# JuliaMolSim/DFTK.jl

Hardware: AMD Instinct MI355X
Metric: SCF iterations/sec (Hψ applies/sec) at fixed Ecut·atoms (higher is better)
Workload: dtype f64

## Files before the change

### dftk.jl_amd/_lib.py

```python
from __future__ import annotations

import ctypes as C
import os

from . import _build

c_cplx_p = C.c_void_p
_i64 = C.c_int64


class dftk_mi_cplx(C.Structure):
    _fields_ = [("re", C.c_double), ("im", C.c_double)]


class dftk_mi_batch_op(C.Structure):
    _fields_ = ([(name, C.c_int32) for name in ("type", "fiber", "trans", "m", "k", "i0", "mode", "flags", "join_next",
                                                 "sync_after", "status", "reserved")] +
                [(name, _i64) for name in ("n", "gm", "gn", "gk", "lda", "ldb", "ldc")] +
                [("alpha", dftk_mi_cplx), ("beta", dftk_mi_cplx), ("s0", C.c_double)] +
                [(name, C.c_void_p) for name in ("A", "B", "W", "W2", "W3", "C", "D", "E", "F", "kb", "host")] +
                [("bytes", C.c_uint64)])


class DftkMiError(RuntimeError):
# ... 87 lines not shown
    "dftk_mi_cube_gradient": (C.c_int, [C.c_void_p, C.c_void_p, C.c_void_p, C.c_void_p]),
    "dftk_mi_xc_gga_spin": (C.c_int, [C.c_void_p, _i64, C.c_void_p, C.c_void_p, C.c_int, C.c_double, C.c_void_p, C.c_void_p,
                                      C.c_void_p]),
    "dftk_mi_symmetrize_rho": (C.c_int, [C.c_void_p, C.c_int, C.c_void_p, C.c_void_p, C.c_int, C.c_void_p, C.c_void_p]),
    "dftk_mi_mix_kerker": (C.c_int, [C.c_void_p, C.c_void_p, C.c_double, C.c_void_p, C.c_void_p]),
    "dftk_mi_mix_dielectric": (C.c_int, [C.c_void_p, C.c_void_p, C.c_double, C.c_double, C.c_void_p, C.c_void_p]),
    "dftk_mi_chi0_dielectric_apply": (C.c_int, [C.c_void_p, C.c_void_p, C.c_double, C.c_double, C.c_void_p, C.c_void_p]),
    "dftk_mi_cube_fourier_filter": (C.c_int, [C.c_void_p, C.c_void_p, C.c_void_p, C.c_void_p]),
    "dftk_mi_kblocks_set_potential": (C.c_int, [C.c_int, C.c_void_p, C.c_void_p]),
    "dftk_mi_lobpcg_multi": (C.c_int, [C.c_int, C.c_void_p, C.c_int, C.c_void_p, C.c_void_p, C.c_double, C.c_int, C.c_int,
                                       C.c_int, C.c_int, C.c_void_p, C.c_void_p, C.c_void_p, C.c_void_p, C.c_void_p,
                                       C.c_void_p, C.c_void_p]),
    "dftk_mi_density_accumulate_multi": (C.c_int, [C.c_int, C.c_void_p, C.c_void_p, C.c_void_p, C.c_void_p, C.c_void_p,
                                                   C.c_void_p]),
    "dftk_mi_density_accumulate_multi2": (C.c_int, [C.c_int, C.c_void_p, C.c_void_p, C.c_void_p, C.c_void_p, C.c_void_p,
                                                    C.c_void_p, C.c_void_p, C.c_void_p]),
    "dftk_mi_band_kinetic_multi": (C.c_int, [C.c_int, C.c_void_p, C.c_void_p, C.c_void_p, C.c_void_p, C.c_void_p]),
    "dftk_mi_batch_stats": (C.c_int, [C.POINTER(_i64), C.POINTER(_i64), C.POINTER(_i64), C.POINTER(_i64)]),
    "dftk_mi_lobpcg_small_stats": (C.c_int, [C.POINTER(_i64), C.POINTER(_i64)]),
    "dftk_mi_ortho_small": (C.c_int, [C.c_void_p, _i64, C.c_int, C.c_void_p, _i64, C.c_int, C.c_void_p, _i64, C.c_void_p,
                                      C.c_double, C.c_void_p]),
    "dftk_mi_batch_replay": (C.c_int, [C.c_void_p, C.c_int, C.c_int, C.c_void_p]),
    "dftk_mi_lobpcg_last_AX": (C.c_void_p, [C.c_void_p]),
    "dftk_mi_lobpcg_history": (C.c_int, [C.c_void_p, C.POINTER(C.c_int), C.POINTER(C.c_int), C.c_void_p, C.c_size_t,
                                         C.POINTER(C.c_int)]),
    "dftk_mi_columnwise_norms": (C.c_int, [C.c_void_p, _i64, C.c_int, C.c_void_p, _i64, C.c_void_p]),
    "dftk_mi_columnwise_dots": (C.c_int, [C.c_void_p, _i64, C.c_int, C.c_void_p, _i64, C.c_void_p, _i64, C.c_void_p]),
    "dftk_mi_ortho_qr": (C.c_int, [C.c_void_p, _i64, C.c_int, C.c_void_p, _i64, C.c_int, C.POINTER(C.c_int),
                                   C.POINTER(C.c_int)]),
    "dftk_mi_tpa_precondprep": (C.c_int, [C.c_void_p, C.c_int, C.c_void_p, _i64, C.c_void_p]),
    "dftk_mi_tpa_ldiv": (C.c_int, [C.c_void_p, C.c_int, C.c_void_p, _i64, C.c_void_p, C.c_double, C.c_void_p, _i64]),
    "dftk_mi_block_residual": (C.c_int, [C.c_void_p, C.c_int, C.c_void_p, _i64, C.c_void_p, _i64, C.c_void_p,
                                         C.c_void_p, _i64, C.c_void_p, C.c_void_p, C.c_void_p]),
    "dftk_mi_kblock_set_gamma_real": (C.c_int, [C.c_void_p, C.c_int]),
    "dftk_mi_gamma_half_size": (C.c_int, [C.c_void_p, C.POINTER(_i64)]),
    "dftk_mi_gamma_tables_host": (C.c_int, [C.c_int, C.c_int, C.c_int, _i64, C.c_void_p, C.POINTER(_i64), C.c_void_p,
                                            C.c_void_p]),
    "dftk_mi_gamma_compress": (C.c_int, [C.c_void_p, C.c_int, C.c_void_p, _i64, C.c_void_p, _i64]),
    "dftk_mi_gamma_compress_aligned": (C.c_int, [C.c_void_p, C.c_int, C.c_void_p, _i64, C.c_void_p, _i64]),
    "dftk_mi_gamma_expand": (C.c_int, [C.c_void_p, C.c_int, C.c_void_p, _i64, C.c_void_p, _i64]),
    "dftk_mi_gamma_apply_H": (C.c_int, [C.c_void_p, C.c_int, C.c_int, C.c_void_p, _i64, C.c_void_p, _i64]),
    "dftk_mi_density_accumulate_real": (C.c_int, [C.c_void_p, C.c_int, C.c_void_p, _i64, C.c_void_p, C.c_void_p]),
    "dftk_mi_shard_plan_host": (C.c_int, [C.c_int, C.c_int, C.c_int, C.c_void_p, C.c_void_p, C.c_void_p, C.c_void_p,
                                          C.c_void_p, C.c_void_p]),
    "dftk_mi_kblock_set_shard": (C.c_int, [C.c_void_p, C.c_void_p, C.c_void_p]),
    "dftk_mi_zgemm": (C.c_int, [C.c_void_p, C.c_char, _i64, _i64, _i64, dftk_mi_cplx, C.c_void_p, _i64,
                                C.c_void_p, _i64, dftk_mi_cplx, C.c_void_p, _i64]),
    "dftk_mi_zgemm_ex": (C.c_int, [C.c_void_p, C.c_char, _i64, _i64, _i64, dftk_mi_cplx, C.c_void_p, _i64,
                                   C.c_void_p, _i64, dftk_mi_cplx, C.c_void_p, _i64, C.c_int]),
    "dftk_mi_zgemm_to": (C.c_int, [C.c_void_p, C.c_char, _i64, _i64, _i64, dftk_mi_cplx, C.c_void_p, _i64,
                                   C.c_void_p, _i64, dftk_mi_cplx, C.c_void_p, _i64, C.c_void_p, C.c_int]),
    "dftk_mi_zgemm_plan_host": (C.c_int, [C.c_char, _i64, _i64, _i64, C.c_int, C.POINTER(C.c_int)]),
    "dftk_mi_zgemm_fold_host": (C.c_int, [C.c_char, _i64, _i64, _i64, C.c_int, C.c_int, C.POINTER(C.c_int), C.POINTER(C.c_int)]),
    "dftk_mi_heev": (C.c_int, [C.c_void_p, C.c_int, C.c_void_p, _i64, C.c_void_p, C.c_void_p, _i64]),
    "dftk_mi_prof_zgemm_shapes": (C.c_int, [C.c_void_p, C.c_int, C.c_void_p, C.c_void_p, C.POINTER(C.c_int)]),
    "dftk_mi_eig_mirror_tall": (C.c_int, [C.c_void_p, C.c_int, C.c_int, C.c_void_p, _i64]),
    "dftk_mi_heev_lowest": (C.c_int, [C.c_void_p, C.c_int, C.c_int, C.c_void_p, _i64, C.c_void_p, C.c_void_p, _i64]),
    "dftk_mi_heev_sigma_host": (C.c_int, [C.c_int, C.c_void_p, C.c_int, C.POINTER(C.c_double), C.POINTER(C.c_double),
                                          C.POINTER(C.c_int), C.c_double]),
    "dftk_mi_potrf_trtri": (C.c_int, [C.c_void_p, C.c_int, C.c_void_p, _i64, C.c_void_p, _i64]),
    "dftk_mi_potrf_trtri_real": (C.c_int, [C.c_void_p, C.c_int, C.c_void_p, _i64, C.c_void_p, _i64]),
    "dftk_mi_lowdin_ortho": (C.c_int, [C.c_void_p, _i64, C.c_int, C.c_void_p, _i64, C.c_void_p]),
    "dftk_mi_pdos_accumulate": (C.c_int, [C.c_void_p, _i64, C.c_int, C.c_void_p, _i64, C.c_int, C.c_void_p, _i64, C.c_void_p,
                                          C.c_double, C.c_int, C.c_double, C.c_int, C.c_void_p, C.c_void_p, C.c_void_p]),
    "dftk_mi_hubbard_occupation": (C.c_int, [C.c_void_p, _i64, C.c_int, C.c_void_p, _i64, C.c_int, C.c_void_p, _i64, C.c_void_p,
                                             C.c_int, C.c_void_p, C.c_void_p, C.c_void_p]),
    "dftk_mi_hubbard_rotate": (C.c_int, [C.c_void_p, _i64, C.c_int, C.c_void_p, C.c_void_p, C.c_void_p, _i64, C.c_void_p,
                                         C.c_void_p, _i64]),
    "dftk_mi_comm_get_unique_id": (C.c_int, [C.c_char_p]),
    "dftk_mi_comm_init_rank": (C.c_int, [C.c_char_p, C.c_int, C.c_int, C.c_int, C.POINTER(C.c_void_p)]),
    "dftk_mi_comm_create_host": (C.c_int, [C.c_int, C.c_int, C.c_int, C.c_void_p, C.c_void_p, C.c_void_p,
                                           C.POINTER(C.c_void_p)]),
    "dftk_mi_comm_destroy": (C.c_int, [C.c_void_p]),
    "dftk_mi_comm_describe": (C.c_int, [C.c_void_p, C.POINTER(C.c_int), C.POINTER(C.c_int), C.POINTER(C.c_int)]),
    "dftk_mi_comm_rank": (C.c_int, [C.c_void_p]),
    "dftk_mi_comm_size": (C.c_int, [C.c_void_p]),
    "dftk_mi_allreduce_sum_f64": (C.c_int, [C.c_void_p, C.c_void_p, C.c_size_t, C.c_void_p]),
    "dftk_mi_prof_enable": (C.c_int, [C.c_void_p, C.c_int]),
    "dftk_mi_prof_get": (C.c_int, [C.c_void_p, C.c_int, C.POINTER(C.c_double), C.POINTER(C.c_double),
                                   C.POINTER(_i64)]),
    "dftk_mi_anderson_create": (C.c_int, [C.c_void_p, _i64, C.c_int, C.c_double, C.c_double, C.POINTER(C.c_void_p)]),
    "dftk_mi_anderson_destroy": (C.c_int, [C.c_void_p]),
    "dftk_mi_anderson_reset": (C.c_int, [C.c_void_p]),
    "dftk_mi_anderson_history": (C.c_int, [C.c_void_p]),
    "dftk_mi_anderson_step": (C.c_int, [C.c_void_p, C.c_void_p, C.c_double, C.c_void_p, C.c_void_p, C.POINTER(C.c_int)]),
    "dftk_mi_chi0_mix": (C.c_int, [C.c_void_p, C.c_int, C.c_void_p, C.c_void_p, C.c_void_p, C.c_double, C.c_int, C.c_double,
                                   C.c_double, C.c_void_p, C.c_double, C.c_int, C.c_int, C.c_void_p, C.POINTER(C.c_int),
                                   C.POINTER(C.c_int)]),
    "dftk_mi_launch_count": (C.c_int, [C.POINTER(_i64), C.POINTER(_i64)]),
    "dftk_mi_device_buffers_live": (C.c_int, [C.POINTER(_i64), C.POINTER(_i64)]),
    "dftk_mi_kblock_reuse_AX": (C.c_int, [C.c_void_p, C.c_int]),
    "dftk_mi_ax_reuse_count": (C.c_int, [C.POINTER(_i64)]),
    "dftk_mi_planes_reuse_count": (C.c_int, [C.POINTER(_i64)]),
    "dftk_mi_step_sums": (C.c_int, [C.c_void_p, _i64, C.c_void_p, C.c_void_p, C.c_void_p, C.c_void_p]),
    "dftk_mi_fermi_bisection": (C.c_int, [C.c_int, C.c_void_p, C.c_void_p, C.c_void_p, C.c_int, C.c_double, C.c_double,
                                          C.c_double, C.c_double, C.c_double, C.POINTER(C.c_double)]),
    "dftk_mi_diag_mfma_peak": (C.c_int, [C.c_void_p, C.c_int, C.c_int, C.POINTER(C.c_double)]),
    "dftk_mi_jacobi_schedule_host": (C.c_int, [C.c_int, C.c_int, C.POINTER(C.c_int), C.POINTER(C.c_int),
                                               C.POINTER(C.c_int)]),
    "dftk_mi_fft_plan_host": (C.c_int, [C.c_int, C.POINTER(C.c_int), C.POINTER(C.c_int), C.POINTER(C.c_int)]),
    "dftk_mi_sphere_tables_host": (C.c_int, [C.c_int, C.c_int, C.c_int, _i64, C.c_void_p, C.POINTER(_i64),
                                             C.POINTER(C.c_int), C.c_void_p, C.c_void_p]),
}

ALLREDUCE_FN = C.CFUNCTYPE(C.c_int, C.c_void_p, C.POINTER(C.c_double), C.c_size_t)
ALLTOALLV_FN = C.CFUNCTYPE(C.c_int, C.c_void_p, C.POINTER(C.c_double), C.POINTER(C.c_size_t), C.POINTER(C.c_size_t),
# ... 38 lines not shown
```

### dftk.jl_amd/csrc/api.cpp

```cpp
#include "common.h"
#include <chrono>
#include "batch.h"
#include <algorithm>
#include <cmath>
#include <cstdarg>
#include <cstdio>
#include <cstdlib>
#include <cstring>
#include <vector>

static thread_local char g_err[1024] = "";

void dftk_set_error(const char* fmt, ...) {
    va_list ap;
    va_start(ap, fmt);
    vsnprintf(g_err, sizeof(g_err), fmt, ap);
    va_end(ap);
}

extern "C" const char* dftk_mi_last_error(void) { return g_err; }

hipError_t dftk_scratch_malloc(void** p, size_t bytes) {
    static const bool poison = getenv("DFTK_MI_POISON") != nullptr;
    hipError_t e = hipMalloc(p, bytes);
// ... 1331 lines not shown
                if (smearing == 2) {
                    f = 0.5 * std::erfc(x);
                } else if (x > 0) {
                    const double y = std::exp(-x);
                    f = y / (1.0 + y);
                } else {
                    f = 1.0 / (1.0 + std::exp(x));
                }
                sk += filled * f;
            }
            total += kweights[k] * sk;
            e += n_bands[k];
        }
        return total - n_electrons;
    };
    for (int it = 0; it < 200; ++it) {
        const double mid = 0.5 * (lo + hi);
        if (mid == lo || mid == hi) break;
        if (excess(mid) < 0)
            lo = mid;
        else
            hi = mid;
    }
    *eF_out = 0.5 * (lo + hi);
    return 0;
}

extern "C" int dftk_mi_kblock_reuse_AX(dftk_mi_kblock* kb, int on) {
    if (!kb) return DFTK_MI_EINVAL;
    kb->ho.promise(on != 0);
    return 0;
}

extern "C" const dftk_mi_cplx* dftk_mi_lobpcg_last_AX(dftk_mi_kblock* kb) {
    return kb ? reinterpret_cast<const dftk_mi_cplx*>(kb->ho.last_AX()) : nullptr;
}

extern "C" int dftk_mi_zgemm(dftk_mi_basis* b, char transA, int64_t m, int64_t n, int64_t k, dftk_mi_cplx alpha,
                             const dftk_mi_cplx* A_d, int64_t lda, const dftk_mi_cplx* B_d, int64_t ldb,
                             dftk_mi_cplx beta, dftk_mi_cplx* C_d, int64_t ldc) {
    if (!b || m < 0 || n < 0 || k < 0 || !C_d) return DFTK_MI_EINVAL;
    HIPCHK(hipSetDevice(b->device));
    cd al = {alpha.re, alpha.im}, be = {beta.re, beta.im};
    return zgemm(b, transA, m, n, k, al, reinterpret_cast<const cd*>(A_d), lda, reinterpret_cast<const cd*>(B_d), ldb,
                 be, reinterpret_cast<cd*>(C_d), ldc);
}

int zgemm_plan_host(char transA, int64_t m, int64_t n, int64_t k, int flags, int* out);
extern "C" int dftk_mi_zgemm_plan_host(char transA, int64_t m, int64_t n, int64_t k, int flags, int* out12) {
    return zgemm_plan_host(transA, m, n, k, flags, out12);
}

int zgemm_fold_host(char transA, int64_t m, int64_t n, int64_t k, int flags, int cap, int* items4, int* count);
extern "C" int dftk_mi_zgemm_fold_host(char transA, int64_t m, int64_t n, int64_t k, int flags, int cap, int* items4, int* count) {
    return zgemm_fold_host(transA, m, n, k, flags, cap, items4, count);
}

extern "C" int dftk_mi_zgemm_ex(dftk_mi_basis* b, char transA, int64_t m, int64_t n, int64_t k, dftk_mi_cplx alpha,
                                const dftk_mi_cplx* A_d, int64_t lda, const dftk_mi_cplx* B_d, int64_t ldb,
                                dftk_mi_cplx beta, dftk_mi_cplx* C_d, int64_t ldc, int flags) {
    if (!b || m < 0 || n < 0 || k < 0 || !C_d || (flags & ~(3 | DFTK_MI_GEMM_REAL | DFTK_MI_GEMM_SYM_RESULT))) return DFTK_MI_EINVAL;
    HIPCHK(hipSetDevice(b->device));
    cd al = {alpha.re, alpha.im}, be = {beta.re, beta.im};
    return zgemm(b, transA, m, n, k, al, reinterpret_cast<const cd*>(A_d), lda, reinterpret_cast<const cd*>(B_d), ldb,
                 be, reinterpret_cast<cd*>(C_d), ldc, flags);
}

extern "C" int dftk_mi_zgemm_to(dftk_mi_basis* b, char transA, int64_t m, int64_t n, int64_t k, dftk_mi_cplx alpha,
                                const dftk_mi_cplx* A_d, int64_t lda, const dftk_mi_cplx* B_d, int64_t ldb,
                                dftk_mi_cplx beta, const dftk_mi_cplx* C_d, int64_t ldc, dftk_mi_cplx* D_d, int flags) {
    if (!b || m < 0 || n < 0 || k < 0 || !C_d || !D_d || (flags & ~(3 | DFTK_MI_GEMM_REAL | DFTK_MI_GEMM_SYM_RESULT)))
        return DFTK_MI_EINVAL;
    HIPCHK(hipSetDevice(b->device));
    cd al = {alpha.re, alpha.im}, be = {beta.re, beta.im};
    return zgemm_to(b, transA, m, n, k, al, reinterpret_cast<const cd*>(A_d), lda, reinterpret_cast<const cd*>(B_d), ldb,
                    be, reinterpret_cast<const cd*>(C_d), ldc, reinterpret_cast<cd*>(D_d), flags);
}

extern "C" int dftk_mi_heev(dftk_mi_basis* b, int n, dftk_mi_cplx* A_d, int64_t lda, double* W_h, dftk_mi_cplx* V_d,
                            int64_t ldv) {
    if (!b || n < 1 || !A_d || !W_h || !V_d || lda < n || ldv < n) return DFTK_MI_EINVAL;
    HIPCHK(hipSetDevice(b->device));
    return dense_heev(b, n, reinterpret_cast<cd*>(A_d), lda, W_h, reinterpret_cast<cd*>(V_d), ldv);
}

extern "C" int dftk_mi_eig_mirror_tall(dftk_mi_basis* b, int n, int real, dftk_mi_cplx* X_d, int64_t ldt) {
    if (!b || n < 1 || !X_d || ldt < (real ? (n + 1) / 2 : n) || 2 * ldt > INT32_MAX) return DFTK_MI_EINVAL;
    HIPCHK(hipSetDevice(b->device));
    return eig_mirror_tall(b, n, real != 0, reinterpret_cast<cd*>(X_d), ldt);
}

extern "C" int dftk_mi_heev_lowest(dftk_mi_basis* b, int n, int nev, dftk_mi_cplx* A_d, int64_t lda, double* W_h,
                                   dftk_mi_cplx* V_d, int64_t ldv) {
    if (!b || n < 1 || nev < 1 || nev > n || !A_d || !W_h || !V_d || lda < n || ldv < n) return DFTK_MI_EINVAL;
    HIPCHK(hipSetDevice(b->device));
    return dense_heev_lowest(b, n, nev, reinterpret_cast<cd*>(A_d), lda, W_h, reinterpret_cast<cd*>(V_d), ldv);
}
extern "C" int dftk_mi_heev_sigma_host(int n, const double* diag_h, int nev, double* sigma, double* gap_guess,
                                       int* hold_iterations, double norm_bound) {
    const int st = eig_choose_sigma_host(n, diag_h, nev, sigma, gap_guess);
    if (st != 0) return st;
    if (hold_iterations) *hold_iterations = norm_bound > 0.0 ? eig_hold_iterations_host(*gap_guess / norm_bound) : 0;
    return 0;
}

extern "C" int dftk_mi_potrf_trtri(dftk_mi_basis* b, int n, dftk_mi_cplx* A_d, int64_t lda, dftk_mi_cplx* invR_d,
// ... 122 lines not shown
```

### dftk.jl_amd/csrc/dense_kernels.hip

```cpp
#include "common.h"
#include "batch.h"
#include "ew_device.h"
#include <algorithm>
#include <atomic>
#include <mutex>
#include <cmath>
#include <numeric>
#include <cstring>
#include <vector>

template <int NT>
__global__ __launch_bounds__(NT) void k_col_reduce(int mode, int64_t n, const cd* __restrict__ X, int64_t ldx,
                                                   const cd* __restrict__ Y, int64_t ldy,
                                                   const double* __restrict__ w, double* __restrict__ out) {
    const int c = blockIdx.x;
    ew_col_reduce<NT>(mode, n, X + (int64_t)c * ldx, Y ? Y + (int64_t)c * ldy : nullptr, w, out + c);
}
template <int NT>
__global__ __launch_bounds__(NT) void k_col_dots2(int64_t n, const cd* __restrict__ X, int64_t ldx, const cd* __restrict__ Y,
                                                  int64_t ldy, double* __restrict__ out_xy, double* __restrict__ out_xx) {
    const int c = blockIdx.x;
    ew_col_dots2<NT>(n, X + (int64_t)c * ldx, Y + (int64_t)c * ldy, out_xy + c, out_xx + c);
}
template <int NT>
// ... 214 lines not shown
            }
        }
        __syncthreads();
        for (int e = t; e < 1024; e += 256) {
            const int k = e >> 5, r = e & 31;
            const int gi = i0 + r, gk = i0 + k;
            Rt[r * 33 + k] = (gi < n && gk < n && r <= k) ? R[gi + (int64_t)gk * ldr] : make_double2(0.0, 0.0);
        }
        __syncthreads();
        for (int k = 31; k >= 0; --k) {
            const int gk = i0 + k;
            if (rr == k) {
                const double d = Rt[k * 33 + k].x;
                Zs[gk * TRI_TC + cc] = (gk < n) ? make_double2(acc.x / d, acc.y / d) : make_double2(0.0, 0.0);
            }
            __syncthreads();
            if (rr < k) {
                const cd zk = Zs[gk * TRI_TC + cc];
                const cd a = Rt[rr * 33 + k];
                acc.x -= a.x * zk.x - a.y * zk.y;
                acc.y -= a.x * zk.y + a.y * zk.x;
            }
        }
    }
    __syncthreads();
    const int ncol = jmax - jc0 + 1;
    for (int e = t; e < n * ncol; e += 256) {
        const int cj = e / n, i = e - cj * n;
        Z[i + (int64_t)(jc0 + cj) * ldz] = (i < 32 * nblk) ? Zs[i * TRI_TC + cj] : make_double2(0.0, 0.0);
    }
}

#define CCB 16
#define CCT 512
__device__ __forceinline__ cd e_mul(cd a, cd b) { return make_double2(a.x * b.x - a.y * b.y, a.x * b.y + a.y * b.x); }
__device__ __forceinline__ cd e_mulc(cd a, cd b) { return make_double2(a.x * b.x + a.y * b.y, a.y * b.x - a.x * b.y); }
__device__ __forceinline__ double e_mul(double a, double b) { return a * b; }
__device__ __forceinline__ double e_mulc(double a, double b) { return a * b; }
__device__ __forceinline__ void e_sub(cd& acc, cd z) { acc.x -= z.x; acc.y -= z.y; }
__device__ __forceinline__ void e_sub(double& acc, double z) { acc -= z; }
__device__ __forceinline__ void e_add(cd& acc, cd z) { acc.x += z.x; acc.y += z.y; }
__device__ __forceinline__ void e_add(double& acc, double z) { acc += z; }
__device__ __forceinline__ cd e_scale(cd a, double s) { return make_double2(a.x * s, a.y * s); }
__device__ __forceinline__ double e_scale(double a, double s) { return a * s; }
__device__ __forceinline__ double e_re(cd a) { return a.x; }
__device__ __forceinline__ double e_re(double a) { return a; }
__device__ __forceinline__ void e_set(cd& dst, double re) { dst = make_double2(re, 0.0); }
__device__ __forceinline__ void e_set(double& dst, double re) { dst = re; }
__device__ __forceinline__ void e_load_conj(cd& dst, cd a, bool diag) { dst = make_double2(a.x, diag ? 0.0 : -a.y); }
__device__ __forceinline__ void e_load_conj(double& dst, cd a, bool) { dst = a.x; }
__device__ __forceinline__ cd e_out_conj(cd a) { return make_double2(a.x, -a.y); }
__device__ __forceinline__ cd e_out_conj(double a) { return make_double2(a, 0.0); }
__device__ __forceinline__ void coop_wait(const int* flag) {
    if (threadIdx.x == 0)
        while (__hip_atomic_load(flag, __ATOMIC_ACQUIRE, __HIP_MEMORY_SCOPE_AGENT) == 0) __builtin_amdgcn_s_sleep(1);
    __syncthreads();
    __threadfence();
}
__device__ __forceinline__ void coop_signal(int* flag) {
    __threadfence();
    __syncthreads();
    if (threadIdx.x == 0) __hip_atomic_store(flag, 1, __ATOMIC_RELEASE, __HIP_MEMORY_SCOPE_AGENT);
}
template <typename T>
__global__ __launch_bounds__(CCT, 1) void k_potrf_trtri_coop(int n, cd* __restrict__ A, int64_t lda, cd* __restrict__ Z,
                                                             int64_t ldz, T* __restrict__ Lbuf, T* __restrict__ Wbuf,
                                                             int* __restrict__ flags, int* __restrict__ info) {
    extern __shared__ __attribute__((aligned(16))) char sm[];
    T* Xs = reinterpret_cast<T*>(sm);
    __shared__ T Dm[CCB][CCB + 1];
    __shared__ T Wm[CCB][CCB + 1];
    __shared__ T Lj[CCB][CCB + 1];
    const int l = blockIdx.x, nb = gridDim.x, tid = threadIdx.x;
    const int r0 = CCB * l;
    const int np = CCB * nb;
    const int nrows = np - r0;
    int* flagsW = flags + 32;
    auto panel = [&](int j) { return Lbuf + (size_t)j * np * CCB; };
    const int i = tid, gr = r0 + i;
    const bool have_row = i < nrows;
    T row[CCB];
#pragma unroll
    for (int c = 0; c < CCB; ++c) {
        const int gc = r0 + c;
        e_set(row[c], 0.0);
        if (have_row) {
            if (gr < n && gc < n) {
                if (gr >= gc) e_load_conj(row[c], A[gc + (int64_t)gr * lda], gr == gc);
            } else if (gr == gc) {
                e_set(row[c], 1.0);
            }
        }
    }
    for (int j = 0; j < l; ++j) {
        coop_wait(flags + j);
        const T* P = panel(j) + (size_t)(r0 - CCB * j) * CCB;
        if (tid < CCB * CCB) Lj[tid >> 4][tid & 15] = P[tid];
        T p[CCB];
        if (have_row) {
#pragma unroll
            for (int t = 0; t < CCB; ++t) p[t] = P[(size_t)i * CCB + t];
        }
        __syncthreads();
        if (have_row) {
#pragma unroll
            for (int c = 0; c < CCB; ++c) {
                T s;
                e_set(s, 0.0);
#pragma unroll
                for (int t = 0; t < CCB; ++t) e_add(s, e_mulc(p[t], Lj[c][t]));
                e_sub(row[c], s);
            }
        }
        __syncthreads();
    }
    if (tid < CCB) {
#pragma unroll
        for (int c = 0; c < CCB; ++c) Dm[tid][c] = row[c];
    }
    __syncthreads();
    if (tid < 64) {
        const int m = tid & 15, kb = tid >> 4;
        for (int c = 0; c < CCB; ++c) {
            const double d = e_re(Dm[c][c]);
            const bool ok = d > 0.0 && isfinite(d);
            if (!ok && tid == 0) atomicCAS(info, 0, r0 + c + 1);
            const double sd = ok ? sqrt(d) : 1.0, inv = 1.0 / sd;
            __builtin_amdgcn_wave_barrier();
            if (m == c) {
#pragma unroll
                for (int q = 0; q < 4; ++q) {
                    const int k = 4 * q + kb;
                    if (k == c)
                        e_set(Dm[k][c], sd);
                    else if (k > c)
                        Dm[k][c] = e_scale(Dm[k][c], inv);
                }
            }
            __builtin_amdgcn_fence(__ATOMIC_RELEASE, "wavefront");
            __builtin_amdgcn_wave_barrier();
            __builtin_amdgcn_fence(__ATOMIC_ACQUIRE, "wavefront");
            if (m > c) {
                const T lm = Dm[m][c];
#pragma unroll
                for (int q = 0; q < 4; ++q) {
                    const int k = 4 * q + kb;
                    if (k >= m) e_sub(Dm[k][m], e_mulc(Dm[k][c], lm));
                }
            }
            __builtin_amdgcn_fence(__ATOMIC_RELEASE, "wavefront");
            __builtin_amdgcn_wave_barrier();
            __builtin_amdgcn_fence(__ATOMIC_ACQUIRE, "wavefront");
        }
#pragma unroll
        for (int q = 0; q < 4; ++q) {
            const int k = 4 * q + kb;
            if (m > k) e_set(Dm[k][m], 0.0);
        }
    }
    __syncthreads();
    if (have_row) {
        if (i < CCB) {
#pragma unroll
            for (int c = 0; c < CCB; ++c) row[c] = Dm[i][c];
        } else {
#pragma unroll
            for (int c = 0; c < CCB; ++c) {
                T acc = row[c];
#pragma unroll
                for (int t = 0; t < CCB; ++t)
                    if (t < c) e_sub(acc, e_mulc(row[t], Dm[c][t]));
                row[c] = e_scale(acc, 1.0 / e_re(Dm[c][c]));
            }
        }
        T* P = panel(l);
#pragma unroll
        for (int c = 0; c < CCB; ++c) P[(size_t)i * CCB + c] = row[c];
    }
    coop_signal(flags + l);
    if (have_row) {
#pragma unroll
        for (int c = 0; c < CCB; ++c) {
            const int gc = r0 + c;
            if (gr < n && gc < n && gr >= gc) A[gc + (int64_t)gr * lda] = e_out_conj(row[c]);
        }
    }
    if (tid < CCB) {
        const int m = tid;
        T w[CCB];
#pragma unroll
        for (int k = 0; k < CCB; ++k) {
            T acc;
            e_set(acc, k == m ? 1.0 : 0.0);
#pragma unroll
            for (int t = 0; t < CCB; ++t)
                if (t < k) e_sub(acc, e_mul(Dm[k][t], w[t]));
            w[k] = e_scale(acc, 1.0 / e_re(Dm[k][k]));
            if (k < m) e_set(w[k], 0.0);
        }
#pragma unroll
        for (int k = 0; k < CCB; ++k) Wm[k][m] = w[k];
    }
    __syncthreads();
    if (tid < CCB * CCB) Wbuf[(size_t)l * CCB * CCB + tid] = Wm[tid >> 4][tid & 15];
    coop_signal(flagsW + l);
    const int a = (tid >> 4) & 15, b = tid & 15, half = tid >> 8;
    if (tid < CCB * CCB) Xs[a * CCB + b] = Wm[a][b];
    __syncthreads();
    for (int k = l + 1; k < nb; ++k) {
        coop_wait(flagsW + k);
        T s;
        e_set(s, 0.0);
        for (int j = l + half; j < k; j += 2) {
            const T* Lkj = panel(j) + (size_t)(CCB * (k - j)) * CCB + a * CCB;
            const T* Xj = Xs + (size_t)(CCB * (j - l)) * CCB + b;
#pragma unroll
            for (int t = 0; t < CCB; ++t) e_add(s, e_mul(Lkj[t], Xj[t * CCB]));
        }
        if (half == 1) Wm[a][b] = s;
        __syncthreads();
        if (half == 0) {
            e_add(s, Wm[a][b]);
            Lj[a][b] = s;
            Dm[a][b] = Wbuf[(size_t)k * CCB * CCB + (tid & 255)];
        }
        __syncthreads();
        if (half == 0) {
            T acc;
            e_set(acc, 0.0);
#pragma unroll
            for (int t = 0; t < CCB; ++t) e_sub(acc, e_mul(Dm[a][t], Lj[t][b]));
            Xs[(size_t)(CCB * (k - l) + a) * CCB + b] = acc;
        }
        __syncthreads();
    }
    for (int e = tid; e < CCB * np; e += CCT) {
        const int bb = e / np, gcol = e - bb * np;
        const int grow = r0 + bb;
        if (grow < n && gcol < n) {
            cd v = make_double2(0.0, 0.0);
            if (gcol >= grow) v = e_out_conj(Xs[(size_t)(gcol - r0) * CCB + bb]);
            Z[grow + (int64_t)gcol * ldz] = v;
        }
    }
}

#define NORMEST_CHUNKS 8
__global__ __launch_bounds__(256) void k_normest_upper(int n, const cd* __restrict__ M, int64_t ldm,
                                                       double* __restrict__ out, const cd* __restrict__ M2,
                                                       int64_t ldm2, double* __restrict__ out2) {
// ... 1142 lines not shown
```

### dftk.jl_amd/csrc/gemm_kernels.hip

```cpp
#include "common.h"
#include "batch.h"
#include <cstdio>
#include <cstdlib>
#include <type_traits>
#include <map>
#include <vector>
#include <cmath>
#include <algorithm>
#include <mutex>

typedef double v4d __attribute__((ext_vector_type(4)));


#define LT_KT 8
#define GEMM_RM 2
#define GEMM_WAVES 4
#define GEMM_BM (GEMM_WAVES * GEMM_RM * 16)
#define M3_RN 2
#define M3_BN (16 * M3_RN)
#define M3_RN_REAL 4
#define M3_BN_REAL (16 * M3_RN_REAL)
#define M3_MIN_BLOCKS 2
__host__ __device__ inline bool gemm_fold_item(int id, int gm, int gn, int* row_t, int* col1, int* col2) {
    const int xcd = id & 7, slot = id >> 3;
    const int np = (gn + 1) >> 1, p = slot % np;
    *row_t = (slot / np) * 8 + xcd;
    *col1 = gn - 1 - p;
    *col2 = (p != gn - 1 - p) ? p : -1;
    return *row_t < gm;
}

template <bool CONJA, int MODE, bool REAL, int RN, bool FOLD = false>
__global__ __launch_bounds__(GEMM_WAVES * 64, M3_MIN_BLOCKS) void k_zgemm_3m(int m, int n, int K, int kchunk, int gm, int gn,
                                                               int rt0, int ct0, int lsplit, int upper,
                                                               int shift_ct, int shift_rt, int nsplit, const cd* __restrict__ A, int64_t lda,
                                                               const cd* __restrict__ B, int64_t ldb,
                                                               const cd* C, cd* D, int64_t ldc, cd alpha, cd beta,
                                                               cd* __restrict__ slab) {
    constexpr int BN = 16 * RN;
    static_assert(RN == 2 || RN == 4, "B staging handles one or two columns per thread");
    __shared__ cd sA[2][LT_KT][GEMM_BM];
    __shared__ cd sB[2][LT_KT][BN];
    const int id = blockIdx.x;
    const int xcd = id & 7, slot = id >> 3;
    int z, row_t, col_t;
    int col2 = -1;
    if (FOLD) {
        if (!gemm_fold_item(id, gm, gn, &row_t, &col_t, &col2)) return;
        z = 0;
    } else if (upper & 16) {
        const int q = (GEMM_BM << ((upper >> 5) & 1)) / BN;
        int L = 0;
        for (int r = 0; r < gm; ++r) L += max(0, gn - r * q);
        const int N = L * nsplit, per = (N + 7) >> 3;
        const int item = xcd * per + slot;
        if (slot >= per || item >= N) return;
        z = item / L;
        int t = item - z * L, r = 0;
        while (t >= gn - r * q) {
            t -= gn - r * q;
            ++r;
        }
        row_t = r;
        col_t = r * q + t;
    } else if (upper & 4) {
        const int per = gm * gn;
        z = (slot / per) * 8 + xcd;
        const int rem = slot % per;
        row_t = rem / gn;
        col_t = rem - row_t * gn;
        if (z >= nsplit) return;
    } else {
        col_t = slot % gn;
        const int R = (slot / gn) * 8 + xcd;
        if (R >= gm * nsplit) return;
        z = R / gm;
        row_t = R - z * gm;
        if (upper & 8) {
            const int g = (gm % 8 == 0) ? 8 : (gm % 4 == 0) ? 4 : (gm % 2 == 0) ? 2 : 1;
            row_t = (row_t + (z * g) / 8) % gm;
        }
    }

    const int tid = threadIdx.x;
    const int lane = tid & 63, wave = tid >> 6;
    const int li = lane & 15, lk = lane >> 4;
    const int tr = lsplit < 0 ? row_t + rt0 : (row_t < lsplit ? row_t : rt0);
    int tcn = lsplit < 0 ? col_t + ct0 : (row_t < lsplit ? ct0 : row_t - lsplit);
    bool shifted = tcn == shift_ct;
    const bool rshifted = tr == shift_rt;
    const int I0 = rshifted ? m - GEMM_BM : tr * GEMM_BM, imin = tr * GEMM_BM;
    int J0 = shifted ? n - BN : tcn * BN, jmin = shifted ? tcn * BN : 0;
    if ((upper & 1) && (imin << ((upper >> 5) & 1)) >= J0 + BN) return;
    const int i0 = I0 + wave * (GEMM_RM * 16);
    const int kbeg = z * kchunk;
    int kend = min(min(K, kbeg + kchunk), (upper & 2) ? J0 + BN : K);
    constexpr bool FULL = MODE == 1;
    const int rmv = FULL ? GEMM_RM : min(GEMM_RM, max(0, (m - i0 + 15) >> 4));
    const int rnv = FULL ? RN : min(RN, max(0, (n - J0 + 15) >> 4));
    const bool active = FULL || (rmv > 0 && rnv > 0);

    v4d acc1[GEMM_RM][RN], acc2[GEMM_RM][RN], acc3[GEMM_RM][RN];
#pragma unroll
    for (int a = 0; a < GEMM_RM; ++a)
#pragma unroll
        for (int b = 0; b < RN; ++b) {
            acc1[a][b] = (v4d){0.0, 0.0, 0.0, 0.0};
            acc2[a][b] = (v4d){0.0, 0.0, 0.0, 0.0};
            acc3[a][b] = (v4d){0.0, 0.0, 0.0, 0.0};
        }

    const int tk = tid & 7, tc = tid >> 3;
    const cd *pA0, *pA1, *pA2, *pA3, *pB0, *pB1;
    auto init_ptrs = [&]() {
        auto a_ptr = [&](int r) -> const cd* {
            if (CONJA) {
                int c = I0 + tc + 32 * r;
// ... 492 lines not shown
    t.gnI = t.gnf + t.shift;
    t.shift_r = (t.gm > t.gmf && t.gmf >= 1) ? 1 : 0;
    t.gmI = t.gmf + t.shift_r;
    t.nright = (t.gnt > t.gnf && !t.shift) ? t.gm : 0;
    t.nbottom = (t.gm > t.gmf && !t.shift_r) ? t.gnI : 0;
    auto live = [&](int tr, int tc) {
        const int64_t jend = (t.shift && tc == t.gnf) ? n : (int64_t)tc * t.BNt + t.BNt;
        return !(upper & 1) || (int64_t)tr * GEMM_BM * rsc < jend;
    };
    std::vector<int> rowsI(t.gmI, 0), rowsB(t.nright + t.nbottom, 0);
    for (int tr = 0; tr < t.gmI; ++tr)
        for (int tc = 0; tc < t.gnI; ++tc) rowsI[tr] += live(tr, tc) ? 1 : 0;
    for (int e = 0; e < t.nright; ++e) rowsB[e] = live(e, t.gnf) ? 1 : 0;
    for (int e = 0; e < t.nbottom; ++e) rowsB[t.nright + e] = live(t.gmf, e) ? 1 : 0;
    bool compact_ok = (upper & 1) && (GEMM_BM * rsc) % t.BNt == 0;
    for (int tr = 0; tr < t.gmI && compact_ok; ++tr)
        compact_ok = rowsI[tr] == std::max(0, t.gnI - tr * (GEMM_BM * rsc / t.BNt));
    t.I = gemm_plan_split(m, n, k, upper, rowsI, false, compact_ok, rsc);
    t.B = gemm_plan_split(m, n, k, upper, rowsB, true, false, rsc);
    return t;
}
bool zgemm_sym_result_pays(int64_t m, int64_t n, int64_t k, bool real) {
    if (m <= 0 || n <= 0 || k <= 0) return false;
    const GemmTiling t = gemm_tiling(m, n, k, 0, real);
    return (int64_t)t.gmI * t.gnI * t.I.nsplit > GEMM_SLOTS;
}

static bool gemm_folds(const GemmTiling& t, bool conja, int upper) {
    return !conja && (upper & 3) == 2 && t.I.nsplit == 1 && !t.I.zmajor && t.gmI >= 1 && t.gnI >= 2;
}
int zgemm_fold_host(char transA, int64_t m, int64_t n, int64_t k, int flags, int cap, int* items4, int* count) {
    if (m <= 0 || n <= 0 || k <= 0 || (flags & ~(3 | DFTK_MI_GEMM_REAL)) || cap < 0 || !count || (cap > 0 && !items4))
        return DFTK_MI_EINVAL;
    const GemmTiling t = gemm_tiling(m, n, k, flags & 3, (flags & DFTK_MI_GEMM_REAL) != 0);
    *count = 0;
    if (!gemm_folds(t, transA == 'C' || transA == 'c', flags & 3)) return 0;
    const int nblk = ((t.gmI + 7) / 8) * 8 * ((t.gnI + 1) / 2);
    for (int id = 0; id < nblk; ++id) {
        int row, c[2];
        if (!gemm_fold_item(id, t.gmI, t.gnI, &row, &c[0], &c[1])) continue;
        for (int i = 0; i < 2; ++i) {
            if (c[i] < 0) continue;
            if (*count < cap) {
                const int64_t j0 = (t.shift && c[i] == t.gnf) ? n - t.BNt : (int64_t)c[i] * t.BNt;
                int* e = items4 + 4 * (int64_t)*count;
                e[0] = row; e[1] = c[i]; e[2] = 0; e[3] = (int)std::min<int64_t>(k, j0 + t.BNt);
            }
            ++*count;
        }
    }
    return 0;
}

int zgemm_plan_host(char transA, int64_t m, int64_t n, int64_t k, int flags, int* out) {
    if (m <= 0 || n <= 0 || k <= 0 || (flags & ~(3 | DFTK_MI_GEMM_REAL | DFTK_MI_GEMM_SYM_RESULT)) || !out) return DFTK_MI_EINVAL;
    (void)transA;
    const bool real = (flags & DFTK_MI_GEMM_REAL) != 0, sym = (flags & DFTK_MI_GEMM_SYM_RESULT) != 0;
    const GemmTiling t = gemm_tiling(m, n, k, (flags & 3) | (sym ? 1 : 0), real, (sym && real) ? 2 : 1);
    const int v[12] = {t.BNt, t.gmf, t.gnf, t.nright, t.nbottom, t.I.nsplit, t.I.kchunk, t.I.compact ? 2 : t.I.zmajor ? 1 : 0,
                       t.B.nsplit, t.B.kchunk, t.B.zmajor ? 1 : 0, t.shift};
    for (int i = 0; i < 12; ++i) out[i] = v[i];
    return 0;
}

int zgemm(dftk_mi_basis* b, char transA, int64_t m, int64_t n, int64_t k, cd alpha, const cd* A, int64_t lda,
          const cd* B, int64_t ldb, cd beta, cd* C, int64_t ldc, int upper_in) {
    return zgemm_to(b, transA, m, n, k, alpha, A, lda, B, ldb, beta, C, ldc, C, upper_in);
}

int zgemm_to(dftk_mi_basis* b, char transA, int64_t m, int64_t n, int64_t k, cd alpha, const cd* A, int64_t lda,
             const cd* B, int64_t ldb, cd beta, const cd* C, int64_t ldc, cd* D, int upper_in) {
    const bool real = (upper_in & DFTK_MI_GEMM_REAL) != 0;
    if (m <= 0 || n <= 0) return 0;
    const bool conja = (transA == 'C' || transA == 'c');
    const bool sym = (upper_in & GEMM_SYM_RESULT) != 0;
    if (sym && conja) {
        dftk_set_error("zgemm: GEMM_SYM_RESULT is a flag of 'N' products");
        return DFTK_MI_EINVAL;
    }
    const int upper = (upper_in & 3) | (sym ? 1 : 0);
    const int rsc = (sym && real) ? 2 : 1;
    if (!conja && !(transA == 'N' || transA == 'n')) {
        dftk_set_error("zgemm: transA must be 'N' or 'C'");
        return DFTK_MI_EINVAL;
    }
    if (m > INT32_MAX || n > INT32_MAX || k > INT32_MAX) return DFTK_MI_EINVAL;
    if (batching()) {
        if (D != C) {
            dftk_set_error("zgemm: a recorded product of a batched call writes its result in place");
            return DFTK_MI_EINVAL;
        }
        BOp o;
        o.b = b;
        o.type = BOP_ZGEMM; o.trans = conja ? 'C' : 'N'; o.gm = m; o.gn = n; o.gk = k; o.alpha = alpha; o.A = A; o.lda = lda;
        o.B = B; o.ldb = ldb; o.beta = beta; o.C = D; o.ldc = ldc;
        o.flags = upper_in & ~GEMM_SYM_RESULT;
        return batch_record(std::move(o));
    }
    if (k <= 0) {
        hipLaunchKernelGGL(k_zgemm_reduce, dim3((unsigned)((m * n + 255) / 256)), dim3(256), 0, b->stream, (int)m,
                           (int)n, (int)m, (int)n, 0, (const cd*)nullptr, 0, (const cd*)nullptr, C, D, ldc, alpha, beta, 0);
        HIPCHK(hipGetLastError());
        return 0;
    }
    static const bool trace = getenv("DFTK_MI_TRACE_GEMM") != nullptr;
    if (trace) fprintf(stderr, "[zgemm] %c %lld %lld %lld\n", transA, (long long)m, (long long)n, (long long)k);
// ... 122 lines not shown
```

### include/dftk_mi355x.h

```cpp
#ifndef DFTK_MI355X_H
#define DFTK_MI355X_H

#include <stddef.h>
#include <stdint.h>

#ifdef __cplusplus
extern "C" {
#endif

typedef struct { double re, im; } dftk_mi_cplx;

typedef struct dftk_mi_basis  dftk_mi_basis;
typedef struct dftk_mi_kblock dftk_mi_kblock;
typedef struct dftk_mi_comm   dftk_mi_comm;

#define DFTK_MI_OK                 0
#define DFTK_MI_EINVAL            (-1)
#define DFTK_MI_EHIP              (-2)
#define DFTK_MI_ERCCL             (-3)
#define DFTK_MI_ENOGPU            (-100)
#define DFTK_MI_NUM_NONFINITE       1
#define DFTK_MI_NUM_CHOLESKY        2
#define DFTK_MI_NUM_NORMALIZATION   3
#define DFTK_MI_NUM_EIGEN           4
// ... 270 lines not shown
int dftk_mi_comm_describe(const dftk_mi_comm* comm, int* backend, int* n_ranks, int* version);
int dftk_mi_comm_rank(const dftk_mi_comm* comm);
int dftk_mi_comm_size(const dftk_mi_comm* comm);
int dftk_mi_allreduce_sum_f64(dftk_mi_comm* comm, double* buf_d, size_t n, void* stream);

int dftk_mi_kblock_set_shard(dftk_mi_kblock* kb, dftk_mi_comm* comm, const int64_t* row_starts_h);

int dftk_mi_kblock_set_gamma_real(dftk_mi_kblock* kb, int on);
int dftk_mi_gamma_half_size(dftk_mi_kblock* kb, int64_t* n_half);
int dftk_mi_gamma_tables_host(int nx, int ny, int nz, int64_t n_G, const int64_t* mapping0_h, int64_t* n_half,
                              int32_t* row_h, int32_t* partner_row_h);
int dftk_mi_gamma_compress(dftk_mi_kblock* kb, int m, const dftk_mi_cplx* X_d, int64_t ldx, dftk_mi_cplx* Xh_d,
                           int64_t ldh);
int dftk_mi_gamma_compress_aligned(dftk_mi_kblock* kb, int m, const dftk_mi_cplx* X_d, int64_t ldx, dftk_mi_cplx* Xh_d,
                                   int64_t ldh);
int dftk_mi_gamma_expand(dftk_mi_kblock* kb, int m, const dftk_mi_cplx* Xh_d, int64_t ldh, dftk_mi_cplx* X_d,
                         int64_t ldx);
int dftk_mi_gamma_apply_H(dftk_mi_kblock* kb, int which, int n_bands, const dftk_mi_cplx* psih_d, int64_t ld_psi,
                          dftk_mi_cplx* Hpsih_d, int64_t ld_Hpsi);
int dftk_mi_density_accumulate_real(dftk_mi_kblock* kb, int n_bands, const dftk_mi_cplx* psi_d, int64_t ld_psi,
                                    const double* weight_h, double* rho_d);

int dftk_mi_shard_plan_host(int n_ranks, int rank, int n_bands, const int64_t* row_starts_h, int* band_starts,
                            int64_t* slab_off, int64_t* slab_cnt, int64_t* band_off, int64_t* band_cnt);

int dftk_mi_prof_enable(dftk_mi_basis* basis, int on);
int dftk_mi_prof_get(dftk_mi_basis* basis, int family, double* total_ms, double* work, int64_t* launches);
typedef struct dftk_mi_anderson dftk_mi_anderson;
int dftk_mi_anderson_create(dftk_mi_basis* basis, int64_t n, int m, double maxcond, double errorfactor,
                            dftk_mi_anderson** out);
int dftk_mi_anderson_destroy(dftk_mi_anderson* acc);
int dftk_mi_anderson_reset(dftk_mi_anderson* acc);
int dftk_mi_anderson_history(const dftk_mi_anderson* acc);
int dftk_mi_anderson_step(dftk_mi_anderson* acc, const double* x_d, double alpha, const double* Pf_d, double* x_next_d,
                          int* n_history );
int dftk_mi_chi0_mix(dftk_mi_kblock* cube_kblock, int n_comp, const double* recip_lattice_h, const double* poisson_d,
                     const double* ldos_d, double dvol, int dielectric, double kTF, double eps_r, const double* dF_d,
                     double reltol, int krylovdim, int maxiter, double* drho_d, int* n_applies, int* converged);

int dftk_mi_launch_count(int64_t* launches, int64_t* host_syncs);

int dftk_mi_device_buffers_live(int64_t* count, int64_t* bytes);

int dftk_mi_step_sums(dftk_mi_basis* basis, int64_t n, const double* a_d, const double* b_d, const double* c_d, double* out_h);

int dftk_mi_fermi_bisection(int n_k, const int* n_bands, const double* eig, const double* kweights, int smearing,
                            double temperature, double filled, double n_electrons, double lo, double hi, double* eF_out);
int dftk_mi_prof_zgemm_shapes(dftk_mi_basis* basis, int cap, int64_t* rows6, double* ms, int* count);

int dftk_mi_diag_mfma_peak(dftk_mi_basis* basis, int waves_per_simd, int iters, double* tflops);

int dftk_mi_zgemm_plan_host(char transA, int64_t m, int64_t n, int64_t k, int flags, int* out12);
int dftk_mi_zgemm_fold_host(char transA, int64_t m, int64_t n, int64_t k, int flags, int cap, int* items4, int* count);
int dftk_mi_jacobi_schedule_host(int n, int round, int* n_blocks, int* pairs ,
                                 int* where );
int dftk_mi_fft_plan_host(int n, int* n_radices, int* radices , int* pos );
int dftk_mi_sphere_tables_host(int nx, int ny, int nz, int64_t n_G, const int64_t* mapping0_h,
                               int64_t* n_lines, int* n_zplanes, int64_t* line_id ,
                               int64_t* line_start );

#ifdef __cplusplus
}
#endif
#endif
```

Measured before the change: 6.306.

## Use wave-register Cholesky in potrf_trtri coop kernel and lighten flag fences

Rewrites the diagonal 16x16 Cholesky block in the cooperative potrf/trtri kernel to work in registers via readlane broadcasts instead of shared-memory updates with wave barriers. It caches reciprocal diagonals in a Dinv array and drops one __syncthreads per panel loop iteration by reordering the shared Lj write. The inter-block flag wait and signal now use relaxed atomics with explicit agent fences in place of full __threadfence. It also factors the compact GEMM tile mapping into a shared host/device helper and exposes it for host inspection, which risks subtle memory-ordering bugs.

Measured after the change: 6.448 (median of 6 runs). 2.3% higher.

```diff
diff --git a/dftk.jl_amd/_lib.py b/dftk.jl_amd/_lib.py
--- a/dftk.jl_amd/_lib.py
+++ b/dftk.jl_amd/_lib.py
@@ -163,6 +163,7 @@
                                    C.c_void_p, _i64, dftk_mi_cplx, C.c_void_p, _i64, C.c_void_p, C.c_int]),
     "dftk_mi_zgemm_plan_host": (C.c_int, [C.c_char, _i64, _i64, _i64, C.c_int, C.POINTER(C.c_int)]),
     "dftk_mi_zgemm_fold_host": (C.c_int, [C.c_char, _i64, _i64, _i64, C.c_int, C.c_int, C.POINTER(C.c_int), C.POINTER(C.c_int)]),
+    "dftk_mi_zgemm_compact_host": (C.c_int, [C.c_int, C.c_int, C.c_int, C.c_int, C.c_int, C.POINTER(C.c_int), C.POINTER(C.c_int)]),
     "dftk_mi_heev": (C.c_int, [C.c_void_p, C.c_int, C.c_void_p, _i64, C.c_void_p, C.c_void_p, _i64]),
     "dftk_mi_prof_zgemm_shapes": (C.c_int, [C.c_void_p, C.c_int, C.c_void_p, C.c_void_p, C.POINTER(C.c_int)]),
     "dftk_mi_eig_mirror_tall": (C.c_int, [C.c_void_p, C.c_int, C.c_int, C.c_void_p, _i64]),
diff --git a/dftk.jl_amd/csrc/api.cpp b/dftk.jl_amd/csrc/api.cpp
--- a/dftk.jl_amd/csrc/api.cpp
+++ b/dftk.jl_amd/csrc/api.cpp
@@ -1407,6 +1407,10 @@
 }
 
 int zgemm_fold_host(char transA, int64_t m, int64_t n, int64_t k, int flags, int cap, int* items4, int* count);
+int zgemm_compact_host(int gm, int gn, int q, int nsplit, int cap, int* items3, int* count);
+extern "C" int dftk_mi_zgemm_compact_host(int gm, int gn, int q, int nsplit, int cap, int* items3, int* count) {
+    return zgemm_compact_host(gm, gn, q, nsplit, cap, items3, count);
+}
 extern "C" int dftk_mi_zgemm_fold_host(char transA, int64_t m, int64_t n, int64_t k, int flags, int cap, int* items4, int* count) {
     return zgemm_fold_host(transA, m, n, k, flags, cap, items4, count);
 }
diff --git a/dftk.jl_amd/csrc/dense_kernels.hip b/dftk.jl_amd/csrc/dense_kernels.hip
--- a/dftk.jl_amd/csrc/dense_kernels.hip
+++ b/dftk.jl_amd/csrc/dense_kernels.hip
@@ -290,16 +290,27 @@
 __device__ __forceinline__ cd e_out_conj(cd a) { return make_double2(a.x, -a.y); }
 __device__ __forceinline__ cd e_out_conj(double a) { return make_double2(a, 0.0); }
 __device__ __forceinline__ void coop_wait(const int* flag) {
-    if (threadIdx.x == 0)
-        while (__hip_atomic_load(flag, __ATOMIC_ACQUIRE, __HIP_MEMORY_SCOPE_AGENT) == 0) __builtin_amdgcn_s_sleep(1);
+    if (threadIdx.x == 0) {
+        while (__hip_atomic_load(flag, __ATOMIC_RELAXED, __HIP_MEMORY_SCOPE_AGENT) == 0) __builtin_amdgcn_s_sleep(1);
+        __builtin_amdgcn_fence(__ATOMIC_ACQUIRE, "agent");
+        asm volatile("s_waitcnt vmcnt(0)" ::: "memory");
+    }
     __syncthreads();
-    __threadfence();
 }
 __device__ __forceinline__ void coop_signal(int* flag) {
-    __threadfence();
+    asm volatile("s_waitcnt vmcnt(0)" ::: "memory");
     __syncthreads();
-    if (threadIdx.x == 0) __hip_atomic_store(flag, 1, __ATOMIC_RELEASE, __HIP_MEMORY_SCOPE_AGENT);
-}
+    if (threadIdx.x == 0) {
+        __builtin_amdgcn_fence(__ATOMIC_RELEASE, "agent");
+        asm volatile("s_waitcnt vmcnt(0)" ::: "memory");
+        __hip_atomic_store(flag, 1, __ATOMIC_RELAXED, __HIP_MEMORY_SCOPE_AGENT);
+    }
+}
+__device__ __forceinline__ double lane_bcast(double v, int l) {
+    const int lo = __builtin_amdgcn_readlane(__double2loint(v), l), hi = __builtin_amdgcn_readlane(__double2hiint(v), l);
+    return __hiloint2double(hi, lo);
+}
+__device__ __forceinline__ cd lane_bcast(cd v, int l) { return make_double2(lane_bcast(v.x, l), lane_bcast(v.y, l)); }
 template <typename T>
 __global__ __launch_bounds__(CCT, 1) void k_potrf_trtri_coop(int n, cd* __restrict__ A, int64_t lda, cd* __restrict__ Z,
                                                              int64_t ldz, T* __restrict__ Lbuf, T* __restrict__ Wbuf,
@@ -308,7 +319,8 @@
     T* Xs = reinterpret_cast<T*>(sm);
     __shared__ T Dm[CCB][CCB + 1];
     __shared__ T Wm[CCB][CCB + 1];
-    __shared__ T Lj[CCB][CCB + 1];
+    __shared__ __attribute__((aligned(16))) T Lj[CCB][CCB];
+    __shared__ double Dinv[CCB];
     const int l = blockIdx.x, nb = gridDim.x, tid = threadIdx.x;
     const int r0 = CCB * l;
     const int np = CCB * nb;
@@ -333,12 +345,15 @@
     for (int j = 0; j < l; ++j) {
         coop_wait(flags + j);
         const T* P = panel(j) + (size_t)(r0 - CCB * j) * CCB;
-        if (tid < CCB * CCB) Lj[tid >> 4][tid & 15] = P[tid];
+        T lj;
+        e_set(lj, 0.0);
+        if (tid < CCB * CCB) lj = P[tid];
         T p[CCB];
         if (have_row) {
 #pragma unroll
             for (int t = 0; t < CCB; ++t) p[t] = P[(size_t)i * CCB + t];
         }
+        if (tid < CCB * CCB) Lj[tid >> 4][tid & 15] = lj;
         __syncthreads();
         if (have_row) {
 #pragma unroll
@@ -350,65 +365,47 @@
                 e_sub(row[c], s);
             }
         }
-        __syncthreads();
-    }
-    if (tid < CCB) {
-#pragma unroll
-        for (int c = 0; c < CCB; ++c) Dm[tid][c] = row[c];
-    }
-    __syncthreads();
+    }
     if (tid < 64) {
-        const int m = tid & 15, kb = tid >> 4;
+        const bool mine = tid < CCB;
+        double my_inv = 1.0;
+#pragma unroll
         for (int c = 0; c < CCB; ++c) {
-            const double d = e_re(Dm[c][c]);
+            const double d = e_re(lane_bcast(row[c], c));
             const bool ok = d > 0.0 && isfinite(d);
             if (!ok && tid == 0) atomicCAS(info, 0, r0 + c + 1);
             const double sd = ok ? sqrt(d) : 1.0, inv = 1.0 / sd;
-            __builtin_amdgcn_wave_barrier();
-            if (m == c) {
-#pragma unroll
-                for (int q = 0; q < 4; ++q) {
-                    const int k = 4 * q + kb;
-                    if (k == c)
-                        e_set(Dm[k][c], sd);
-                    else if (k > c)
-                        Dm[k][c] = e_scale(Dm[k][c], inv);
-                }
-            }
-            __builtin_amdgcn_fence(__ATOMIC_RELEASE, "wavefront");
-            __builtin_amdgcn_wave_barrier();
-            __builtin_amdgcn_fence(__ATOMIC_ACQUIRE, "wavefront");
-            if (m > c) {
-                const T lm = Dm[m][c];
-#pragma unroll
-                for (int q = 0; q < 4; ++q) {
-                    const int k = 4 * q + kb;
-                    if (k >= m) e_sub(Dm[k][m], e_mulc(Dm[k][c], lm));
-                }
-            }
-            __builtin_amdgcn_fence(__ATOMIC_RELEASE, "wavefront");
-            __builtin_amdgcn_wave_barrier();
-            __builtin_amdgcn_fence(__ATOMIC_ACQUIRE, "wavefront");
-        }
-#pragma unroll
-        for (int q = 0; q < 4; ++q) {
-            const int k = 4 * q + kb;
-            if (m > k) e_set(Dm[k][m], 0.0);
+            if (tid == c) {
+                e_set(row[c], sd);
+                my_inv = inv;
+            } else if (mine && tid > c) {
+                row[c] = e_scale(row[c], inv);
+            }
+#pragma unroll
+            for (int m = c + 1; m < CCB; ++m) {
+                const T lm = lane_bcast(row[c], m);
+                if (mine && tid >= m) e_sub(row[m], e_mulc(row[c], lm));
+            }
+        }
+        if (mine) {
+#pragma unroll
+            for (int m = 0; m < CCB; ++m) {
+                if (m > tid) e_set(row[m], 0.0);
+                Dm[tid][m] = row[m];
+            }
+            Dinv[tid] = my_inv;
         }
     }
     __syncthreads();
     if (have_row) {
-        if (i < CCB) {
-#pragma unroll
-            for (int c = 0; c < CCB; ++c) row[c] = Dm[i][c];
-        } else {
+        if (i >= CCB) {
 #pragma unroll
             for (int c = 0; c < CCB; ++c) {
                 T acc = row[c];
 #pragma unroll
                 for (int t = 0; t < CCB; ++t)
                     if (t < c) e_sub(acc, e_mulc(row[t], Dm[c][t]));
-                row[c] = e_scale(acc, 1.0 / e_re(Dm[c][c]));
+                row[c] = e_scale(acc, Dinv[c]);
             }
         }
         T* P = panel(l);
@@ -433,7 +430,7 @@
 #pragma unroll
             for (int t = 0; t < CCB; ++t)
                 if (t < k) e_sub(acc, e_mul(Dm[k][t], w[t]));
-            w[k] = e_scale(acc, 1.0 / e_re(Dm[k][k]));
+            w[k] = e_scale(acc, Dinv[k]);
             if (k < m) e_set(w[k], 0.0);
         }
 #pragma unroll
diff --git a/dftk.jl_amd/csrc/gemm_kernels.hip b/dftk.jl_amd/csrc/gemm_kernels.hip
--- a/dftk.jl_amd/csrc/gemm_kernels.hip
+++ b/dftk.jl_amd/csrc/gemm_kernels.hip
@@ -28,6 +28,24 @@
     *col1 = gn - 1 - p;
     *col2 = (p != gn - 1 - p) ? p : -1;
     return *row_t < gm;
+}
+
+__host__ __device__ inline bool gemm_compact_item(int id, int gm, int gn, int q, int nsplit, int* z, int* row_t, int* col_t) {
+    const int xcd = id & 7, slot = id >> 3;
+    int L = 0;
+    for (int r = 0; r < gm; ++r) L += (gn - r * q > 0) ? gn - r * q : 0;
+    const int N = L * nsplit, per = (N + 7) >> 3;
+    const int item = xcd * per + slot;
+    if (slot >= per || item >= N) return false;
+    *z = item / L;
+    int t = item - *z * L, r = 0;
+    while (t >= gn - r * q) {
+        t -= gn - r * q;
+        ++r;
+    }
+    *row_t = r;
+    *col_t = r * q + t;
+    return true;
 }
 
 template <bool CONJA, int MODE, bool REAL, int RN, bool FOLD = false>
@@ -50,19 +68,7 @@
         z = 0;
     } else if (upper & 16) {
         const int q = (GEMM_BM << ((upper >> 5) & 1)) / BN;
-        int L = 0;
-        for (int r = 0; r < gm; ++r) L += max(0, gn - r * q);
-        const int N = L * nsplit, per = (N + 7) >> 3;
-        const int item = xcd * per + slot;
-        if (slot >= per || item >= N) return;
-        z = item / L;
-        int t = item - z * L, r = 0;
-        while (t >= gn - r * q) {
-            t -= gn - r * q;
-            ++r;
-        }
-        row_t = r;
-        col_t = r * q + t;
+        if (!gemm_compact_item(id, gm, gn, q, nsplit, &z, &row_t, &col_t)) return;
     } else if (upper & 4) {
         const int per = gm * gn;
         z = (slot / per) * 8 + xcd;
@@ -661,6 +667,25 @@
     return 0;
 }
 
+int zgemm_compact_host(int gm, int gn, int q, int nsplit, int cap, int* items3, int* count) {
+    if (gm <= 0 || gn <= 0 || q <= 0 || nsplit <= 0 || cap < 0 || !count || (cap > 0 && !items3)) return DFTK_MI_EINVAL;
+    int64_t live = 0;
+    for (int r = 0; r < gm; ++r) live += std::max(0, gn - r * q);
+    const int64_t nblk = ((live * nsplit + 7) / 8) * 8;
+    if (nblk > INT32_MAX) return DFTK_MI_EINVAL;
+    *count = 0;
+    for (int id = 0; id < (int)nblk; ++id) {
+        int z, row, col;
+        if (!gemm_compact_item(id, gm, gn, q, nsplit, &z, &row, &col)) continue;
+        if (*count < cap) {
+            int* e = items3 + 3 * (int64_t)*count;
+            e[0] = z; e[1] = row; e[2] = col;
+        }
+        ++*count;
+    }
+    return 0;
+}
+
 int zgemm_plan_host(char transA, int64_t m, int64_t n, int64_t k, int flags, int* out) {
     if (m <= 0 || n <= 0 || k <= 0 || (flags & ~(3 | DFTK_MI_GEMM_REAL | DFTK_MI_GEMM_SYM_RESULT)) || !out) return DFTK_MI_EINVAL;
     (void)transA;
diff --git a/include/dftk_mi355x.h b/include/dftk_mi355x.h
--- a/include/dftk_mi355x.h
+++ b/include/dftk_mi355x.h
@@ -346,6 +346,7 @@
 
 int dftk_mi_zgemm_plan_host(char transA, int64_t m, int64_t n, int64_t k, int flags, int* out12);
 int dftk_mi_zgemm_fold_host(char transA, int64_t m, int64_t n, int64_t k, int flags, int cap, int* items4, int* count);
+int dftk_mi_zgemm_compact_host(int gm, int gn, int q, int nsplit, int cap, int* items3, int* count);
 int dftk_mi_jacobi_schedule_host(int n, int round, int* n_blocks, int* pairs ,
                                  int* where );
 int dftk_mi_fft_plan_host(int n, int* n_radices, int* radices , int* pos );
```
